# KamilSJaron/smudgeplot

Hardware: NVIDIA H100
Metric: k-mers/sec scanned (hetmers) at 1/2/4/8 H100; bit-exact .smu vs ref C (higher is better)
Workload: dtype u64

## Files before the change

### smudgeplot_b200/csrc/hm_symm.cu

```cuda
#include <cuda_runtime.h>
#include <stdint.h>
#include <stdio.h>
#include <stdlib.h>
#include <string.h>

#include "hetmers_b200.h"
#include "hm_internal.h"
#include "hm_device.cuh"

#define RS_THREADS 256
#define RS_EPT     8
#define RS_TILE    (RS_THREADS*RS_EPT)
#define RS_HALO    64
#define RS_WIN     (RS_TILE+2*RS_HALO)
#define RS_SCANCAP RS_HALO
#define RS_RUNCAP  (RS_HALO+1)
#define RS_LONGRUN 32
#ifndef RS_MINBLOCKS
#define RS_MINBLOCKS 5
#endif
#ifndef RS_STAGE
#define RS_STAGE   384
#endif

#define SY_STATUS_ASYMMETRIC 1ull
#define SY_STATUS_OVERFLOW   2ull

#define SY_HDR_CAND   0
#define SY_HDR_STATUS 1
#define SY_HDR_RUNS   2
#define SY_HDR_S      3
#define SY_HDR_PEND   4
#define SY_HDR_QUERY  5

struct SymmView
  { unsigned long long *cand_n;
    unsigned long long *status;
    uint32_t *bloom;
    uint32_t  seg_words;
    int       n_seg, self;
    uint64_t  first_key[HM_MAX_SHARDS];
    uint64_t *cand_key, *cand_lo, *cand_meta;
    unsigned long long cand_cap;
    unsigned long long *runs_n;
    uint64_t *runs;
    unsigned long long runs_cap;
    uint64_t *s_key, *s_lo;
    unsigned long long s_cap;
    const hm_stream_sview *sviews;
    uint64_t *pend, *pend_key, *pend_lo;
    uint64_t *q_key, *q_lo, *q_tag;
    unsigned long long pend_cap, q_cap;
  };

template <int KW>
__device__ __forceinline__ void bloom_slot(const SymmView &W, int seg, int kmer, uint64_t hi, uint64_t lo,
                                           uint64_t *&word, uint64_t &mask)
{ const int Pr = kmer >> 1, pup = kmer-Pr;
  uint64_t sfx;
  if (KW == 1)
    sfx = hi >> (64-2*kmer);
  else
    { const int sr = 128-2*kmer;
      sfx = sr == 0 ? lo : ((lo >> sr) | (hi << (64-sr)));
    }
  if (2*Pr < 64)
    sfx &= (((uint64_t) 1 << (2*Pr)) - 1);
  const uint64_t pfx = hi >> (64-2*pup);
  uint32_t h = ((uint32_t) sfx ^ (uint32_t) (sfx >> 32) * 0x85EBCA6Bu) * 0x9E3779B1u;
  uint32_t g = ((uint32_t) pfx ^ (uint32_t) (pfx >> 32) * 0xC2B2AE35u) * 0x27D4EB2Fu;
  h ^= h >> 15;
  word = (uint64_t *) (W.bloom + (size_t) seg * W.seg_words) + __umulhi(h * 0x2C1B3C6Du,W.seg_words >> 1);
  mask = (1ull << (g >> 26)) | (1ull << ((g >> 20) & 63)) | (1ull << ((g >> 14) & 63));
}

__device__ __forceinline__ uint64_t ld_keep(const uint64_t *p)
{ uint64_t v, pol;
  asm volatile("createpolicy.fractional.L2::evict_last.b64 %0, 1.0;" : "=l"(pol));
  asm volatile("ld.global.nc.L1::no_allocate.L2::cache_hint.u64 %0, [%1], %2;" : "=l"(v) : "l"(p), "l"(pol));
  return v;
}

__device__ __forceinline__ uint64_t ld_stream(const uint64_t *p)
{ uint64_t v, pol;
  asm volatile("createpolicy.fractional.L2::evict_first.b64 %0, 1.0;" : "=l"(pol));
  asm volatile("ld.global.nc.L1::no_allocate.L2::cache_hint.u64 %0, [%1], %2;" : "=l"(v) : "l"(p), "l"(pol));
  return v;
}

__device__ __forceinline__ void red_or64(uint64_t *p, uint64_t v)
{ asm volatile("red.global.relaxed.gpu.or.b64 [%0], %1;" :: "l"(__cvta_generic_to_global(p)), "l"(v) : "memory"); }

__device__ __forceinline__ int owner_of(const SymmView &W, uint64_t hi)
{ int r = 0;
  for (int s = 1; s < W.n_seg; s++)
    r += (hi >= W.first_key[s]);
  return r;
}

template <typename IdxT, int KW>
__device__ __noinline__ void neighbours_slow(const uint64_t *__restrict__ keys, const uint64_t *__restrict__ keys_lo,
                                             const uint16_t *__restrict__ cnt, const IdxT *__restrict__ bucket,
                                             int bshift, int kmer, int p0, int pup,
                                             uint64_t x, uint64_t xl, int cx,
                                             int &H, int &U, int64_t &part, int &ppos)
{ H = 0; U = 0; part = -1; ppos = 0;
  for (int p = p0; p < kmer; p++)
    { int b = base_at<KW>(x,xl,p);
      for (int c = 0; c < 4; c++)
        { if (c == b) continue;
          uint64_t y = x, yl = xl;
          set_base<KW>(y,yl,p,c);
          int64_t j = bucket_find<IdxT,KW>(keys,keys_lo,bucket,bshift,y,yl);
          if (j >= 0 && cx + (int) __ldg(cnt+j) <= HM_SMAX)
            { H += 1;
              if (p >= pup) U += 1;
              part = j; ppos = p;
            }
        }
    }
}


__device__ __forceinline__ uint64_t fp_mix(uint64_t hi, uint64_t lo, uint32_t c, uint64_t seed)
{ uint64_t v = (hi ^ seed) * 0xBF58476D1CE4E5B9ull;
  v ^= v >> 32;
  v = (v + lo + ((uint64_t) c << 40) + c) * 0x94D049BB133111EBull;
  v ^= v >> 29;
  v *= (seed | 1);
  v ^= v >> 32;
  return v;
}

template <int KW>
__global__ void __launch_bounds__(256)
symm_fingerprint_kernel(const uint64_t *__restrict__ keys, const uint64_t *__restrict__ keys_lo,
                        const uint16_t *__restrict__ cnt, int64_t i0, int64_t i1, int kmer,
                        uint64_t seed0, uint64_t seed1, unsigned long long *__restrict__ acc)
{ uint64_t a0 = 0, a1 = 0, a2 = 0, a3 = 0;
  const int64_t stride = (int64_t) gridDim.x * blockDim.x;
  for (int64_t i = i0 + (int64_t) blockIdx.x * blockDim.x + threadIdx.x; i < i1; i += stride)
    { uint64_t x = keys[i], xl = KW == 2 ? keys_lo[i] : 0, r, rl;
      uint32_t c = cnt[i];
      revcomp_kmer<KW>(x,xl,kmer,r,rl);
      a0 += fp_mix(x,xl,c,seed0);  a1 += fp_mix(x,xl,c,seed1);
      a2 += fp_mix(r,rl,c,seed0);  a3 += fp_mix(r,rl,c,seed1);
    }
  for (int o = 16; o > 0; o >>= 1)
    { a0 += __shfl_xor_sync(0xffffffffu,a0,o); a1 += __shfl_xor_sync(0xffffffffu,a1,o);
      a2 += __shfl_xor_sync(0xffffffffu,a2,o); a3 += __shfl_xor_sync(0xffffffffu,a3,o);
    }
  if ((threadIdx.x & 31) == 0)
    { atomicAdd(acc+0,(unsigned long long) a0); atomicAdd(acc+1,(unsigned long long) a1);
      atomicAdd(acc+2,(unsigned long long) a2); atomicAdd(acc+3,(unsigned long long) a3);
    }
}

extern "C" int hm_k_symm_fingerprint(const uint64_t *d_keys, const uint64_t *d_keys_lo, const uint16_t *d_cnt,
                                     int64_t i0, int64_t i1, int kmer, const uint64_t seed[2],
                                     uint64_t *d_acc, void *stream)
{ if (kmer < 1 || kmer > HM_MAX_KMER || (kmer > 32) != (d_keys_lo != NULL) || seed == NULL || d_acc == NULL)
    return hm_set_error(HM_EINVAL,"symm_fingerprint: bad arguments (k=%d)",kmer);
  if (i1 <= i0)
    return HM_OK;
  int64_t want = (i1-i0+255)/256;
  int     grid = (int) (want < 132*16 ? want : 132*16);
  if (kmer <= 32)
    symm_fingerprint_kernel<1><<<grid,256,0,(cudaStream_t) stream>>>
        (d_keys,NULL,d_cnt,i0,i1,kmer,seed[0],seed[1],(unsigned long long *) d_acc);
  else
    symm_fingerprint_kernel<2><<<grid,256,0,(cudaStream_t) stream>>>
        (d_keys,d_keys_lo,d_cnt,i0,i1,kmer,seed[0],seed[1],(unsigned long long *) d_acc);
// ... 43 lines not shown
  at = (at+255) & ~255ll;
  out->off_cand_key = at;   at += 8*cap;
  out->off_cand_lo = at;    at += (kmer > 32) ? 8*cap : 0;
  out->off_cand_meta = at;  at += 8*cap;
  out->cand_cap = cap;
  out->off_runs = at;       out->runs_cap = range/3 + 1024;   at += 8*out->runs_cap;
  out->n_seg = n_seg;
  out->range = range;
  out->bytes = (at+255) & ~255ll;
  return HM_OK;
}

static void bloom_window(cudaStream_t st, const void *base, size_t bytes, int on)
{ static int limit_set[64] = {0};
  static size_t max_win[64] = {0}, max_persist[64] = {0};
  int dev = 0;
  cudaGetDevice(&dev);
  if (dev < 0 || dev >= 64) return;
  if (!limit_set[dev])
    { cudaDeviceProp p;
      limit_set[dev] = 1;
      if (cudaGetDeviceProperties(&p,dev) == cudaSuccess)
        { max_win[dev] = (size_t) p.accessPolicyMaxWindowSize;
          max_persist[dev] = (size_t) p.persistingL2CacheMaxSize;
          if (max_persist[dev] > 0)
            cudaDeviceSetLimit(cudaLimitPersistingL2CacheSize,max_persist[dev]);
        }
      cudaGetLastError();
    }
  if (max_win[dev] == 0 || max_persist[dev] == 0)
    return;
  cudaStreamAttrValue a;
  memset(&a,0,sizeof(a));
  if (on)
    { size_t w = bytes < max_win[dev] ? bytes : max_win[dev];
      a.accessPolicyWindow.base_ptr  = (void *) base;
      a.accessPolicyWindow.num_bytes = w;
      a.accessPolicyWindow.hitRatio  = w <= max_persist[dev] ? 1.0f : (float) max_persist[dev] / (float) w;
      a.accessPolicyWindow.hitProp   = cudaAccessPropertyPersisting;
      a.accessPolicyWindow.missProp  = cudaAccessPropertyStreaming;
    }
  cudaStreamSetAttribute(st,cudaStreamAttributeAccessPolicyWindow,&a);
  cudaGetLastError();
}

static int l2_persist(void)
{ const char *e = getenv("HETMERS_L2_PERSIST");
  return (e == NULL || strcmp(e,"0") != 0);
}

static SymmView make_view(void *d_work, const hm_symm_layout *L, const hm_symm_shards *sh)
{ SymmView W;
  uint8_t *b = (uint8_t *) d_work;
  memset(&W,0,sizeof(W));
  W.cand_n    = (unsigned long long *) (b + L->off_header) + SY_HDR_CAND;
  W.status    = W.cand_n + SY_HDR_STATUS;
  W.bloom     = (uint32_t *) (b + L->off_bloom);
  W.seg_words = (uint32_t) L->seg_words;
  W.n_seg     = L->n_seg;
  W.self      = 0;
  if (sh != NULL && sh->n_seg > 1)
    { W.self = sh->self;
      for (int r = 0; r < sh->n_seg; r++) W.first_key[r] = sh->first_key[r];
    }
  W.cand_key  = (uint64_t *) (b + L->off_cand_key);
  W.cand_lo   = (uint64_t *) (b + L->off_cand_lo);
  W.cand_meta = (uint64_t *) (b + L->off_cand_meta);
  W.cand_cap  = (unsigned long long) L->cand_cap;
  W.runs_n    = W.cand_n + SY_HDR_RUNS;
  W.runs      = (uint64_t *) (b + L->off_runs);
  W.runs_cap  = (unsigned long long) L->runs_cap;
  return W;
}


template <int KW> struct RsSmem
  { uint64_t *key, *klo;
    uint16_t *cnt;
    uint64_t *ckey, *clo, *cmeta;
    uint16_t *t1;
    uint16_t *t2r;
  };

__device__ __forceinline__ uint64_t pack_meta(int cx, int cy, int pos, int yb)
{ return (uint64_t) cx | ((uint64_t) cy << 16) | ((uint64_t) pos << 32) | ((uint64_t) yb << 40); }

#ifdef RS_PROBE
__device__ int rs_probe_mode;
#define RS_PROBE_IS(m) (rs_probe_mode == (m))
#else
#define RS_PROBE_IS(m) false
#endif

template <int KW>
__device__ __forceinline__ void stage_candidates(const RsSmem<KW> &S, unsigned *s_nc, const SymmView &W,
                                                 bool emit, uint64_t x, uint64_t xl, uint64_t meta,
                                                 int lane, unsigned lt)
{ const unsigned bal = __ballot_sync(0xffffffffu,emit);
  if (bal == 0 || RS_PROBE_IS(4))
    return;
  unsigned base = 0;
  if (lane == 0)
    base = atomicAdd(s_nc,(unsigned) __popc(bal));
  base = __shfl_sync(0xffffffffu,base,0);
  const unsigned at = base + __popc(bal & lt);
  const bool     over = emit && (at >= RS_STAGE);
  if (emit && !over)
    { S.ckey[at] = x;
      if (KW == 2) S.clo[at] = xl;
      S.cmeta[at] = meta;
    }
  if (base + __popc(bal) <= RS_STAGE)
    return;
  const unsigned ob = __ballot_sync(0xffffffffu,over);
  unsigned long long g0 = 0;
  if (lane == 0)
    g0 = atomicAdd(W.cand_n,(unsigned long long) __popc(ob));
  g0 = __shfl_sync(0xffffffffu,g0,0) + (unsigned long long) __popc(ob & lt);
  if (over)
    { if (g0 < W.cand_cap)
        { W.cand_key[g0] = x;
          if (KW == 2) W.cand_lo[g0] = xl;
          W.cand_meta[g0] = meta;
        }
      else
        atomicOr(W.status,SY_STATUS_OVERFLOW);
    }
}

template <int KW>
__device__ __forceinline__ void s_push(const SymmView &W, uint64_t x, uint64_t xl)
{ const unsigned m = __activemask();
  const int      lane = threadIdx.x & 31, lead = __ffs(m)-1;
  unsigned long long at = 0;
  if (lane == lead)
    at = atomicAdd(W.cand_n + SY_HDR_S,(unsigned long long) __popc(m));
  at = __shfl_sync(m,at,lead) + (unsigned long long) __popc(m & ((1u << lane)-1));
  if (at < W.s_cap)
    { W.s_key[at] = x;
      if (KW == 2) W.s_lo[at] = xl;
    }
  else
    atomicOr(W.status,SY_STATUS_OVERFLOW);
}

template <int KW, bool SL>
__device__ __forceinline__ void bloom_insert(const SymmView &W, int kmer, uint64_t x, uint64_t xl)
{ uint64_t *word, mask;
  bloom_slot<KW>(W,W.self,kmer,x,xl,word,mask);
  if (!RS_PROBE_IS(3) || mask == (uint64_t) (uintptr_t) word)
    red_or64(word,mask);
  if (SL)
    s_push<KW>(W,x,xl);
}

template <typename IdxT, int KW, bool SL>
__global__ void __launch_bounds__(256)
runs_kernel(const uint64_t *__restrict__ keys, const uint64_t *__restrict__ keys_lo,
            const uint16_t *__restrict__ cnt, int64_t n, const IdxT *__restrict__ bucket, int bshift,
            int kmer, int64_t lo, int64_t hi, const SymmView W)
{ const int      Pr = kmer >> 1, pup = kmer-Pr, psh = 64-2*Pr;
  const uint64_t pmask = ~(uint64_t) 0 << psh;
  const unsigned FULL = 0xffffffffu;
  const int      lane = threadIdx.x & 31;
  const unsigned lt   = (1u << lane) - 1;
  unsigned long long nrl = *W.runs_n;
  if (nrl > W.runs_cap) nrl = W.runs_cap;
  const int64_t nr     = (int64_t) nrl;
  const int64_t stride = (int64_t) gridDim.x * blockDim.x;
  for (int64_t r0 = (int64_t) blockIdx.x * blockDim.x + threadIdx.x - lane; r0 < nr; r0 += stride)
    { const int64_t r = r0+lane;
      const bool    valid = (r < nr);
      int64_t  h = 0;
      uint64_t x0 = 0;
      if (valid)
        { h  = (int64_t) W.runs[r];
          x0 = __ldg(keys+h);
        }
      unsigned lb = __ballot_sync(FULL,valid);
      while (lb != 0)
        { const int     src = __ffs(lb)-1;
          lb &= lb-1;
          const int64_t hh = __shfl_sync(FULL,h,src);
          const uint64_t xx = __shfl_sync(FULL,x0,src);
          int64_t end = hh+1;
          while (true)
            { const int64_t t = end+lane;
              const bool same = (t < n) && (((__ldg(keys+t) ^ xx) & pmask) == 0);
              const unsigned sb = __ballot_sync(FULL,same);
              if (sb == FULL) { end += 32; continue; }
              end += __ffs(~sb)-1;
              break;
            }
          for (int64_t g0 = hh; g0 < end; g0 += 32)
            { const int64_t g = g0+lane;
              bool     emit = false;
              uint64_t x = 0, xl = 0, meta = 0;
              if (g < end && g >= lo && g < hi)
                { x = __ldg(keys+g);
                  if (KW == 2) xl = __ldg(keys_lo+g);
                  const int cx = __ldg(cnt+g);
                  int Hn, Un, ppos; int64_t part;
                  neighbours_slow<IdxT,KW>(keys,keys_lo,cnt,bucket,bshift,kmer,Pr,pup,x,xl,cx,Hn,Un,part,ppos);
                  if (Un > 0)
                    bloom_insert<KW,SL>(W,kmer,x,xl);
                  if (Hn == 1 && part > g)
                    { const uint64_t y = __ldg(keys+part), yl = KW == 2 ? __ldg(keys_lo+part) : 0;
                      const int cy = __ldg(cnt+part);
                      int Hy, Uy, py; int64_t party;
                      neighbours_slow<IdxT,KW>(keys,keys_lo,cnt,bucket,bshift,kmer,Pr,pup,y,yl,cy,Hy,Uy,party,py);
                      if (Hy == 1)
                        { emit = true;
                          meta = pack_meta(cx,cy,ppos,base_at<KW>(y,yl,ppos));
                        }
                    }
                }
              const unsigned eb = __ballot_sync(FULL,emit);
              if (eb != 0)
                { unsigned long long base = 0;
                  if (lane == 0)
                    base = atomicAdd(W.cand_n,(unsigned long long) __popc(eb));
                  base = __shfl_sync(FULL,base,0) + (unsigned long long) __popc(eb & lt);
                  if (emit)
                    { if (base < W.cand_cap)
                        { W.cand_key[base] = x;
                          if (KW == 2) W.cand_lo[base] = xl;
                          W.cand_meta[base] = meta;
                        }
                      else
                        atomicOr(W.status,SY_STATUS_OVERFLOW);
                    }
                }
            }
        }
    }
}

template <int KW> struct RunSfx    { typedef uint64_t T; };
template <>       struct RunSfx<1> { typedef uint32_t T; };

template <int KW>
__device__ __forceinline__ typename RunSfx<KW>::T run_sfx(uint64_t hi, uint64_t lo, int Pr)
{ if constexpr (KW == 1)
    return (uint32_t) ((hi << 2*Pr) >> 32);
  else
    return (hi << (2*Pr-32) << 32) | (lo >> (64-2*Pr));
}

template <typename T>
__device__ __forceinline__ bool one_base_in_run(T d, int Pr, int &pos)
{ const T u = (d | (d >> 1)) & (T) HM_M5;
  if constexpr (sizeof(T) == 4) pos = Pr + (__clz((int) d) >> 1);
  else                          pos = Pr + (__clzll((long long) d) >> 1);
  return (u & (u-1)) == 0;
}

template <int KW, bool SL, int LMAX>
__device__ __forceinline__ bool settle_members(const RsSmem<KW> &S, const SymmView &W, int kmer, int Pr, int pup,
                                               int h, int L, int a, bool in, bool own, int lane,
                                               uint64_t &x, uint64_t &xl, uint64_t &meta)
{ int Hx = 0, Ux = 0, part = 0, ppos = 0, cx = 0;
  if (in)
    { x  = S.key[h+a];
      xl = KW == 2 ? S.klo[h+a] : 0;
      cx = S.cnt[h+a];
      auto mate = [&](int b)
        { int pos;
          if (b < L && b != a && one_base_in_run(run_sfx<KW>(x ^ S.key[h+b],KW == 2 ? xl ^ S.klo[h+b] : 0,Pr),Pr,pos) &&
              cx + (int) S.cnt[h+b] <= HM_SMAX)
            { Hx += 1;
              if (pos >= pup) Ux += 1;
              part = b; ppos = pos;
            }
        };
      if constexpr (LMAX > 0)
        {
#pragma unroll
          for (int b = 0; b < LMAX; b++)
            mate(b);
        }
      else
        for (int b = 0; b < L; b++)
          mate(b);
      if (own && Ux > 0)
        bloom_insert<KW,SL>(W,kmer,x,xl);
    }
  const int pl = lane + part - a;
  int       Hy = __shfl_sync(0xffffffffu,Hx,pl & 31);
  if (!in || !own || Hx != 1 || part < a)
    return false;
  const uint64_t y = S.key[h+part], yl = KW == 2 ? S.klo[h+part] : 0;
  const int      cy = S.cnt[h+part];
  if (pl > 31)
    { Hy = 0;
      for (int b = 0; b < L; b++)
        { int pos;
          if (b != part && one_base_in_run(run_sfx<KW>(y ^ S.key[h+b],KW == 2 ? yl ^ S.klo[h+b] : 0,Pr),Pr,pos) &&
              cy + (int) S.cnt[h+b] <= HM_SMAX)
            Hy += 1;
        }
    }
  if (Hy != 1)
    return false;
  meta = pack_meta(cx,cy,ppos,base_at<KW>(y,yl,ppos));
  return true;
}

#ifdef RS_PROBE
#define RS_PHASES 6
#define RS_PROBE_SLOTS 1024
__device__ unsigned long long rs_probe_cycles[RS_PROBE_SLOTS*RS_PHASES];
#define RS_PROBE_TILE(b)  (rs_probe_mode == 2 ? (b) % 64 : (b))
#define RS_PROBE_START    long long rs_t = clock64(); unsigned long long rs_acc[RS_PHASES] = {0, 0, 0, 0, 0, 0};
#define RS_PROBE_MARK(ph) { const long long t_ = clock64(); rs_acc[ph] += (unsigned long long) (t_ - rs_t); rs_t = t_; }
#define RS_PROBE_FLUSH()  { if (lane == 0) _Pragma("unroll") for (int p_ = 0; p_ < RS_PHASES; p_++) \
                              atomicAdd(rs_probe_cycles + (blockIdx.x % RS_PROBE_SLOTS)*RS_PHASES + p_,rs_acc[p_]); }
#define RS_PROBE_LOADONLY() if (rs_probe_mode == 1) { RS_PROBE_FLUSH(); return; }

extern "C" int hm_probe_runscan(int mode, unsigned long long *cycles)
{ static unsigned long long rows[RS_PROBE_SLOTS*RS_PHASES];
  cudaError_t e = cudaDeviceSynchronize();
  if (e == cudaSuccess && cycles != NULL)
    { e = cudaMemcpyFromSymbol(rows,rs_probe_cycles,sizeof(rows));
      for (int p = 0; p < RS_PHASES; p++)
        { cycles[p] = 0;
          for (int r = 0; r < RS_PROBE_SLOTS; r++)
            cycles[p] += rows[r*RS_PHASES+p];
        }
    }
  memset(rows,0,sizeof(rows));
  if (e == cudaSuccess)
    e = cudaMemcpyToSymbol(rs_probe_cycles,rows,sizeof(rows));
  if (e == cudaSuccess)
    e = cudaMemcpyToSymbol(rs_probe_mode,&mode,sizeof(mode));
  return e == cudaSuccess ? HM_OK : hm_cuda_fail(e,"hm_probe_runscan");
}
#else
#define RS_PROBE_TILE(b)  (b)
#define RS_PROBE_START
#define RS_PROBE_MARK(ph)
#define RS_PROBE_FLUSH()
#define RS_PROBE_LOADONLY()
#endif

template <typename IdxT, int KW, bool SL>
__global__ void __launch_bounds__(RS_THREADS,RS_MINBLOCKS)
runscan_kernel(const uint64_t *__restrict__ keys, const uint64_t *__restrict__ keys_lo,
               const uint16_t *__restrict__ cnt, int64_t n, const IdxT *__restrict__ bucket, int bshift,
               int kmer, int64_t lo, int64_t hi, int64_t tile0, int use_tma, const SymmView W)
{ extern __shared__ __align__(128) uint8_t smem[];
  __shared__ __align__(8) uint64_t s_bar;
  __shared__ unsigned s_nc, s_nr, s_done;
  RsSmem<KW> S;
  S.key   = (uint64_t *) smem;
  S.klo   = S.key + (KW == 2 ? RS_WIN : 0);
  S.ckey  = S.key + KW*RS_WIN;
  S.clo   = S.ckey + (KW == 2 ? RS_STAGE : 0);
  S.cmeta = S.ckey + KW*RS_STAGE;
  S.cnt   = (uint16_t *) (S.cmeta + RS_STAGE);
  S.t1    = S.cnt + RS_WIN;
  S.t2r   = S.t1 + RS_TILE/2;

  const int      Pr   = kmer >> 1;
  const int      pup  = kmer - Pr;
  const int      psh  = 64-2*Pr;
  const uint64_t pmask = ~(uint64_t) 0 << psh;
  const unsigned FULL = 0xffffffffu;
  const int      lane = threadIdx.x & 31;
  const int      warp = threadIdx.x >> 5;
  const unsigned lt   = (1u << lane) - 1;
  RS_PROBE_START

  const int64_t T0 = (tile0 + RS_PROBE_TILE(blockIdx.x)) * RS_TILE;
  const int64_t ws = T0 - RS_HALO;
  const int64_t e0 = ws > 0 ? ws : 0;
  const int64_t e1 = T0+RS_TILE+RS_HALO < n ? T0+RS_TILE+RS_HALO : n;
  const int     v0 = (int) (e0-ws), v1 = (int) (e1-ws);

  const int m   = v1-v0;
  const int mt  = use_tma ? (m & ~7) : 0;
  if (threadIdx.x == 0)
    { s_nc = 0; s_nr = 0; s_done = 0;
      if (mt > 0)
        { mbar_init(&s_bar,1);
          fence_proxy_async_smem();
        }
    }
  __syncthreads();
  if (threadIdx.x == 0 && mt > 0)
    { mbar_arrive_expect_tx(&s_bar,(unsigned) (mt*(8*KW+2)));
      bulk_copy_g2s(S.key+v0,keys+e0,(unsigned) (8*mt),&s_bar);
      if (KW == 2)
        bulk_copy_g2s(S.klo+v0,keys_lo+e0,(unsigned) (8*mt),&s_bar);
      bulk_copy_g2s(S.cnt+v0,cnt+e0,(unsigned) (2*mt),&s_bar);
    }
  if (mt < m || v0 > 0 || v1 < RS_WIN)
    { for (int j = mt + threadIdx.x; j < m; j += RS_THREADS)
        { S.key[v0+j] = keys[e0+j];
          if (KW == 2) S.klo[v0+j] = keys_lo[e0+j];
          S.cnt[v0+j] = cnt[e0+j];
        }
      if (mt > 0)
        mbar_wait(&s_bar,0);
      __syncthreads();
      const uint64_t sa = ~S.key[v0], sb = ~S.key[v1-1];
      __syncthreads();
      for (int j = threadIdx.x; j < RS_WIN; j += RS_THREADS)
        if (j < v0)       S.key[j] = sa;
        else if (j >= v1) S.key[j] = sb;
      __syncthreads();
    }
  else
    mbar_wait(&s_bar,0);
  RS_PROBE_MARK(0)
  RS_PROBE_LOADONLY()

  const int wd0 = RS_HALO/32 + warp*RS_EPT;
  unsigned  eqw = 0;
#pragma unroll
  for (int t = 0; t < RS_EPT+2; t++)
    { const int i = (wd0-1+t)*32 + lane;
      bool eq;
      if (psh >= 32)
        { const uint32_t a = (uint32_t) (S.key[i] >> 32);
          uint32_t       b = __shfl_down_sync(FULL,a,1);
          if (lane == 31) b = (uint32_t) (S.key[i+1] >> 32);
          eq = (((a ^ b) >> (psh-32)) == 0);
        }
      else
        eq = (((S.key[i] ^ S.key[i+1]) & pmask) == 0);
      const unsigned bal = __ballot_sync(FULL,eq);
      if (lane == t) eqw = bal;
    }
  RS_PROBE_MARK(1)

  const int a0 = RS_HALO + (lo > T0 ? (int) (lo-T0 < RS_TILE ? lo-T0 : RS_TILE) : 0);
  const int a1 = RS_HALO + (hi-T0 < RS_TILE ? (int) (hi-T0) : RS_TILE);
  uint16_t *my1  = S.t1  + warp*(RS_TILE/2/(RS_THREADS/32));
  int n1, n3;
  { const unsigned P = __shfl_up_sync(FULL,eqw,1), N = __shfl_down_sync(FULL,eqw,1);
    unsigned m2 = 0, m3 = 0;
    const int wd = wd0-1+lane;
    if (lane >= 1 && lane <= RS_EPT)
      { const unsigned E = eqw;
        const unsigned em1 = (E << 1) | (P >> 31);
        const unsigned em2 = (E << 2) | (P >> 30);
        const unsigned ep1 = (E >> 1) | (N << 31);
        const int      s0  = wd*32;
        unsigned act = 0xffffffffu;
        if (s0 < a0)      act &= (a0-s0 >= 32) ? 0u : (0xffffffffu << (a0-s0));
        if (s0+32 > a1)   act &= (a1-s0 <= 0)  ? 0u : (0xffffffffu >> (s0+32-a1));
        const unsigned more = (em1 & E) | (E & ep1) | (em1 & em2);
        m2 = (E & ~em1 & ~ep1) & act;
        m3 = more & act & ~em1;
      }
    const int c2 = __popc(m2), c3 = __popc(m3);
    int pre2 = c2, pre3 = c3;
#pragma unroll
    for (int o = 1; o <= RS_EPT; o <<= 1)
      { int v2 = __shfl_up_sync(FULL,pre2,o), v3 = __shfl_up_sync(FULL,pre3,o);
        if (lane >= o) { pre2 += v2; pre3 += v3; }
      }
    n1 = __shfl_sync(FULL,pre2,RS_EPT);
    n3 = __shfl_sync(FULL,pre3,RS_EPT);
    int at = pre2-c2;
    while (m2 != 0)
      { my1[at++] = (uint16_t) (wd*32 + __ffs(m2)-1);
        m2 &= m2-1;
      }
    at = n1 + pre3-c3;
    while (m3 != 0)
      { my1[at++] = (uint16_t) (wd*32 + __ffs(m3)-1);
        m3 &= m3-1;
      }
  }
  __syncwarp();
  if (RS_PROBE_IS(5))
    n3 = 0;
  RS_PROBE_MARK(2)

  for (int i0 = 0; i0 < n1; i0 += 32)
    { const int i = i0+lane;
      bool     emit = false;
      uint64_t x = 0, xl = 0, meta = 0;
      if (i < n1)
        { const int w = my1[i];
          x = S.key[w];
          const uint64_t y = S.key[w+1];
          uint64_t yl = 0;
          if (KW == 2) { xl = S.klo[w]; yl = S.klo[w+1]; }
          const int cx = S.cnt[w], cy = S.cnt[w+1];
          int pos;
          if (one_base_in_run(run_sfx<KW>(x ^ y,xl ^ yl,Pr),Pr,pos) && cx+cy <= HM_SMAX)
            { emit = true;
              meta = pack_meta(cx,cy,pos,base_at<KW>(y,yl,pos));
              if (pos >= pup)
                { bloom_insert<KW,SL>(W,kmer,x,xl);
                  bloom_insert<KW,SL>(W,kmer,y,yl);
                }
            }
        }
      stage_candidates<KW>(S,&s_nc,W,emit,x,xl,meta,lane,lt);
    }
  RS_PROBE_MARK(3)

  const int b1 = hi-T0 < RS_TILE+RS_HALO ? RS_HALO + (int) (hi-T0) : RS_WIN;
  for (int i0 = 0; i0 < n3; i0 += 32)
    { const int i = i0+lane;
      const int h = i < n3 ? my1[n1+i] : 0;
      int       L = 0;
      {
        const int      t  = (h >> 5) - (wd0-1);
        const unsigned w0 = __shfl_sync(FULL,eqw,t & 31), w1 = __shfl_sync(FULL,eqw,(t+1) & 31);
        const unsigned up = __funnelshift_r(w0,w1,h & 31);
        if (i < n3)
          L = (~up != 0) ? __ffs((int) ~up) : 33;
      }
      const int Ls = L <= 8 ? L : 0;
      int inc = Ls;
#pragma unroll
      for (int o = 1; o < 32; o <<= 1)
        { const int v = __shfl_up_sync(FULL,inc,o);
          if (lane >= o) inc += v;
        }
      const int M = __shfl_sync(FULL,inc,31);
      for (int t0 = 0; t0 < M; t0 += 32)
        { const int t = t0+lane;
          int r = 0;
#pragma unroll
          for (int s = 16; s > 0; s >>= 1)
            if (__shfl_sync(FULL,inc,r+s-1) <= t) r += s;
          const int hr = __shfl_sync(FULL,h,r), Lr = __shfl_sync(FULL,Ls,r);
          const int a  = t - (__shfl_sync(FULL,inc,r) - Lr);
          bool     emit = false;
          uint64_t x = 0, xl = 0, meta = 0;
          emit = settle_members<KW,SL,8>(S,W,kmer,Pr,pup,hr,Lr,a,t < M,hr+a < b1,lane,x,xl,meta);
          stage_candidates<KW>(S,&s_nc,W,emit,x,xl,meta,lane,lt);
        }
      unsigned lb = __ballot_sync(FULL,L > 8);
      while (lb != 0)
        { const int src = __ffs(lb)-1;
          lb &= lb-1;
          const int hh = __shfl_sync(FULL,h,src);
          int       LL = __shfl_sync(FULL,L,src);
          if (LL > 32)
            { const uint64_t xh = S.key[hh];
              while (LL <= RS_RUNCAP)
                { const int      t = hh+LL+lane;
                  const unsigned sb = __ballot_sync(FULL,t < RS_WIN && ((S.key[t] ^ xh) & pmask) == 0);
                  if (sb != FULL) { LL += __ffs(~sb)-1; break; }
                  LL += 32;
                }
            }
          if (LL > RS_RUNCAP || hh+LL >= RS_WIN)
            { if (lane == 0)
                S.t2r[atomicAdd(&s_nr,1u)] = (uint16_t) hh;
              continue;
            }
          for (int a0 = 0; a0 < LL; a0 += 32)
            { const int a = a0+lane;
              bool     emit = false;
              uint64_t x = 0, xl = 0, meta = 0;
              emit = settle_members<KW,SL,0>(S,W,kmer,Pr,pup,hh,LL,a,a < LL,hh+a < b1,lane,x,xl,meta);
              stage_candidates<KW>(S,&s_nc,W,emit,x,xl,meta,lane,lt);
            }
        }
    }
  RS_PROBE_MARK(4)

  __syncwarp();
  unsigned last = 0;
  if (lane == 0)
    { __threadfence_block();
      last = (atomicAdd(&s_done,1u) == RS_THREADS/32-1);
    }
  last = __shfl_sync(FULL,last,0);
  if (!last || RS_PROBE_IS(4))
    { RS_PROBE_MARK(5) RS_PROBE_FLUSH() return; }
  __threadfence_block();
  const unsigned nr = s_nr;
  if (nr > 0)
    { unsigned long long rb = 0;
      if (lane == 0)
        rb = atomicAdd(W.runs_n,(unsigned long long) nr);
      rb = __shfl_sync(FULL,rb,0);
      for (unsigned i = lane; i < nr; i += 32)
        if (rb+i < W.runs_cap)
          W.runs[rb+i] = (uint64_t) (T0 + ((int) S.t2r[i] - RS_HALO));
        else
          atomicOr(W.status,SY_STATUS_OVERFLOW);
    }
  const unsigned nc = s_nc < RS_STAGE ? s_nc : RS_STAGE;
  if (nc == 0)
    { RS_PROBE_MARK(5) RS_PROBE_FLUSH() return; }
  unsigned long long base = 0;
  if (lane == 0)
    base = atomicAdd(W.cand_n,(unsigned long long) nc);
  base = __shfl_sync(FULL,base,0);
  for (unsigned i = lane; i < nc; i += 32)
    { unsigned long long at = base + i;
      if (at < W.cand_cap)
        { W.cand_key[at] = S.ckey[i];
          if (KW == 2) W.cand_lo[at] = S.clo[i];
          W.cand_meta[at] = S.cmeta[i];
        }
      else
        atomicOr(W.status,SY_STATUS_OVERFLOW);
    }
  RS_PROBE_MARK(5)
  RS_PROBE_FLUSH()
}

template <typename IdxT, int KW, bool SL>
__global__ void __launch_bounds__(RS_THREADS,RS_MINBLOCKS)
runscan_dense_kernel(const uint64_t *__restrict__ keys, const uint64_t *__restrict__ keys_lo,
                     const uint16_t *__restrict__ cnt, int64_t n, int kmer, int64_t lo, int64_t hi,
                     int64_t tile0, int use_tma, const SymmView W)
{ extern __shared__ __align__(128) uint8_t smem[];
  __shared__ __align__(8) uint64_t s_bar;
  __shared__ unsigned s_nc, s_nl, s_done;
  __shared__ unsigned s_eq[RS_WIN/32+1];
  RsSmem<KW> S;
  S.key   = (uint64_t *) smem;
  S.klo   = S.key + (KW == 2 ? RS_WIN : 0);
  S.ckey  = S.key + KW*RS_WIN;
  S.clo   = S.ckey + (KW == 2 ? RS_STAGE : 0);
  S.cmeta = S.ckey + KW*RS_STAGE;
  S.cnt   = (uint16_t *) (S.cmeta + RS_STAGE);
  S.t1    = S.cnt + RS_WIN;
  S.t2r   = S.t1 + RS_WIN;
  uint16_t *s_part = S.t2r + RS_TILE/8;
  unsigned *hu = (unsigned *) (s_part + RS_WIN);
  uint32_t *rem = hu + RS_WIN/2;

  const int      Pr   = kmer >> 1, pup = kmer - Pr, psh = 64-2*Pr;
  const uint64_t pmask = ~(uint64_t) 0 << psh;
  const unsigned FULL = 0xffffffffu;
  const int      lane = threadIdx.x & 31;
  const int      warp = threadIdx.x >> 5;
  const unsigned lt   = (1u << lane) - 1;

  const int64_t T0 = (tile0 + blockIdx.x) * RS_TILE;
  const int64_t ws = T0 - RS_HALO;
  const int64_t e0 = ws > 0 ? ws : 0;
  const int64_t e1 = T0+RS_TILE+RS_HALO < n ? T0+RS_TILE+RS_HALO : n;
  const int     v0 = (int) (e0-ws), v1 = (int) (e1-ws);

  const int m   = v1-v0;
  const int mt  = use_tma ? (m & ~7) : 0;
  if (threadIdx.x == 0)
    { s_nc = 0; s_nl = 0; s_done = 0;
      if (mt > 0)
        { mbar_init(&s_bar,1);
          fence_proxy_async_smem();
        }
    }
  for (int j = threadIdx.x; j < RS_WIN/2; j += RS_THREADS)
    hu[j] = 0;
  __syncthreads();
  if (threadIdx.x == 0 && mt > 0)
    { mbar_arrive_expect_tx(&s_bar,(unsigned) (mt*(8*KW+2)));
      bulk_copy_g2s(S.key+v0,keys+e0,(unsigned) (8*mt),&s_bar);
      if (KW == 2)
        bulk_copy_g2s(S.klo+v0,keys_lo+e0,(unsigned) (8*mt),&s_bar);
      bulk_copy_g2s(S.cnt+v0,cnt+e0,(unsigned) (2*mt),&s_bar);
    }
  if (mt < m || v0 > 0 || v1 < RS_WIN)
    { for (int j = mt + threadIdx.x; j < m; j += RS_THREADS)
        { S.key[v0+j] = keys[e0+j];
          if (KW == 2) S.klo[v0+j] = keys_lo[e0+j];
          S.cnt[v0+j] = cnt[e0+j];
        }
      if (mt > 0)
        mbar_wait(&s_bar,0);
      __syncthreads();
      const uint64_t sa = ~S.key[v0], sb = ~S.key[v1-1];
      __syncthreads();
      for (int j = threadIdx.x; j < RS_WIN; j += RS_THREADS)
        if (j < v0)       S.key[j] = sa;
        else if (j >= v1) S.key[j] = sb;
      __syncthreads();
    }
  else
    mbar_wait(&s_bar,0);

  const bool narrow = (KW == 1) && (kmer-Pr <= 16);
  for (int wd = warp; wd < RS_WIN/32; wd += RS_THREADS/32)
    { const int i = wd*32 + lane;
      bool eq = false;
      const uint64_t ki = S.key[i];
      if (i+1 < RS_WIN)
        eq = (((ki ^ S.key[i+1]) & pmask) == 0);
      if (narrow)
        rem[i] = (uint32_t) ((ki << (2*Pr)) >> 32);
      const unsigned bal = __ballot_sync(FULL,eq);
      if (lane == 0)
        s_eq[wd] = bal;
    }
  if (threadIdx.x == 0)
    s_eq[RS_WIN/32] = 0;
  __syncthreads();

  const int a0 = RS_HALO + (lo > T0 ? (int) (lo-T0 < RS_TILE ? lo-T0 : RS_TILE) : 0);
  const int a1 = RS_HALO + (hi-T0 < RS_TILE ? (int) (hi-T0) : RS_TILE);
  for (int i = threadIdx.x; i < RS_WIN; i += RS_THREADS)
    { const int      w = i >> 5, b = i & 31;
      const unsigned up = __funnelshift_r(s_eq[w],s_eq[w+1],b);
      const int      fwd = (~up == 0) ? 32 : __ffs((int) ~up)-1;
      int back = 0;
      if (i > 0)
        { const int      wq = (i-1) >> 5, bq = (i-1) & 31;
          const unsigned dn = __funnelshift_l(wq > 0 ? s_eq[wq-1] : 0u,s_eq[wq],31-bq);
          back = (~dn == 0) ? 32 : __clz((int) ~dn);
        }
      uint16_t mark = (uint16_t) fwd;
      if (back+fwd+1 > RS_LONGRUN)
        { mark = 0xffff;
          if (back == 0 && i >= a0 && i < a1)
            S.t2r[atomicAdd(&s_nl,1u)] = (uint16_t) i;
        }
      S.t1[i] = mark;
      s_part[i] = (uint16_t) i;
    }
  __syncthreads();

  for (int i = threadIdx.x; i < RS_WIN; i += RS_THREADS)
    { const int fwd = S.t1[i];
      if (fwd == 0 || fwd == 0xffff)
        continue;
      const int cx = S.cnt[i];
      if (narrow)
        { const uint32_t rx = rem[i];
          for (int j = i+1; j <= i+fwd; j++)
            { const uint32_t d = rx ^ rem[j];
              const uint32_t u = (d | (d>>1)) & 0x55555555u;
              if ((u & (u-1)) == 0 && cx + (int) S.cnt[j] <= HM_SMAX)
                { const int      pos = Pr + (__clz((int) d) >> 1);
                  const unsigned inc = 1u | (pos >= pup ? 0x100u : 0u);
                  atomicAdd(hu + (i>>1), inc << (16*(i&1)));
                  atomicAdd(hu + (j>>1), inc << (16*(j&1)));
                  s_part[i] = (uint16_t) j;
                  s_part[j] = (uint16_t) i;
                }
            }
        }
      else
        { const uint64_t x = S.key[i], xl = KW == 2 ? S.klo[i] : 0;
          for (int j = i+1; j <= i+fwd; j++)
            { int pos;
              if (one_base_apart<KW>(x,xl,S.key[j],KW == 2 ? S.klo[j] : 0,pos) && cx + (int) S.cnt[j] <= HM_SMAX)
                { const unsigned inc = 1u | (pos >= pup ? 0x100u : 0u);
                  atomicAdd(hu + (i>>1), inc << (16*(i&1)));
                  atomicAdd(hu + (j>>1), inc << (16*(j&1)));
                  s_part[i] = (uint16_t) j;
                  s_part[j] = (uint16_t) i;
                }
            }
        }
    }
  __syncthreads();

  for (int i0 = RS_HALO + (threadIdx.x & ~31); i0 < RS_HALO+RS_TILE; i0 += RS_THREADS)
    { const int i = i0+lane;
      bool     emit = false;
      uint64_t x = 0, xl = 0, meta = 0;
      if (i >= a0 && i < a1 && S.t1[i] != 0xffff)
        { const unsigned c = (hu[i>>1] >> (16*(i&1))) & 0xffffu;
          const int H = (int) (c & 0xff), U = (int) (c >> 8);
          if (H > 0)
            { x = S.key[i];
              if (KW == 2) xl = S.klo[i];
              if (U > 0)
                bloom_insert<KW,SL>(W,kmer,x,xl);
              const int j = s_part[i];
              if (H == 1 && j > i && ((hu[j>>1] >> (16*(j&1))) & 0xffu) == 1)
                { const uint64_t y = S.key[j], yl = KW == 2 ? S.klo[j] : 0;
                  int pos;
                  one_base_apart<KW>(x,xl,y,yl,pos);
                  emit = true;
                  meta = pack_meta(S.cnt[i],S.cnt[j],pos,base_at<KW>(y,yl,pos));
                }
            }
        }
      stage_candidates<KW>(S,&s_nc,W,emit,x,xl,meta,lane,lt);
    }

  __syncwarp();
  unsigned last = 0;
  if (lane == 0)
    { __threadfence_block();
      last = (atomicAdd(&s_done,1u) == RS_THREADS/32-1);
    }
  last = __shfl_sync(FULL,last,0);
  if (!last)
    return;
  __threadfence_block();
  const unsigned nr = s_nl;
  if (nr > 0)
    { unsigned long long rb = 0;
      if (lane == 0)
        rb = atomicAdd(W.runs_n,(unsigned long long) nr);
      rb = __shfl_sync(FULL,rb,0);
      for (unsigned i = lane; i < nr; i += 32)
        if (rb+i < W.runs_cap)
          W.runs[rb+i] = (uint64_t) (T0 + ((int) S.t2r[i] - RS_HALO));
        else
          atomicOr(W.status,SY_STATUS_OVERFLOW);
    }
  const unsigned nc = s_nc < RS_STAGE ? s_nc : RS_STAGE;
  if (nc == 0)
    return;
  unsigned long long base = 0;
  if (lane == 0)
    base = atomicAdd(W.cand_n,(unsigned long long) nc);
  base = __shfl_sync(FULL,base,0);
  for (unsigned i = lane; i < nc; i += 32)
    { unsigned long long at = base + i;
      if (at < W.cand_cap)
        { W.cand_key[at] = S.ckey[i];
          if (KW == 2) W.cand_lo[at] = S.clo[i];
          W.cand_meta[at] = S.cmeta[i];
        }
      else
        atomicOr(W.status,SY_STATUS_OVERFLOW);
    }
}

template <typename I, int K> struct Inst { typedef I IdxT; static constexpr int KW = K; };

template <class F>
static cudaError_t dispatch(int kmer, int idx64, F f)
{ if (kmer <= 32)
    return idx64 ? f(Inst<uint64_t,1>()) : f(Inst<uint32_t,1>());
  return idx64 ? f(Inst<uint64_t,2>()) : f(Inst<uint32_t,2>());
}

template <typename IdxT, int KW, bool SL = false>
static cudaError_t launch_runscan(const uint64_t *keys, const uint64_t *keys_lo, const uint16_t *cnt, int64_t n,
                                  const void *bucket, int bits, int kmer, int64_t lo, int64_t hi,
                                  const SymmView &W, cudaStream_t st)
{ static int configured[64] = {0};
  int dev = 0;
  cudaGetDevice(&dev);
  int64_t tile0 = lo/RS_TILE, tile1 = (hi+RS_TILE-1)/RS_TILE;
  int     tma   = ((((uintptr_t) keys) | ((uintptr_t) cnt) | ((uintptr_t) (keys_lo ? keys_lo : keys))) & 15) == 0;
  const int   Pr  = kmer >> 1;
  double      lam = (2*Pr >= 62) ? 0.0 : (double) n / (double) ((uint64_t) 1 << (2*Pr));
  bool        dense = (lam > 0.6);
  const char *force = getenv("HETMERS_RUNSCAN");
  if (force != NULL && strcmp(force,"dense") == 0)  dense = true;
  if (force != NULL && strcmp(force,"sparse") == 0) dense = false;
  cudaError_t e;
  if (dense)
    { size_t smem = (size_t) RS_WIN*(8*KW+2) + (size_t) RS_STAGE*8*(KW+1) +
                    2*(size_t) (RS_WIN+RS_TILE/8+RS_WIN) + 4*(size_t) (RS_WIN/2+RS_WIN);
      if (smem > 48*1024 && (dev >= 64 || !(configured[dev] & 2)))
        { e = cudaFuncSetAttribute(runscan_dense_kernel<IdxT,KW,SL>,cudaFuncAttributeMaxDynamicSharedMemorySize,(int) smem);
          if (e != cudaSuccess) return e;
          if (dev < 64) configured[dev] |= 2;
        }
      runscan_dense_kernel<IdxT,KW,SL><<<(unsigned) (tile1-tile0),RS_THREADS,smem,st>>>
          (keys,keys_lo,cnt,n,kmer,lo,hi,tile0,tma,W);
    }
  else
    { size_t smem = (size_t) RS_WIN*(8*KW+2) + (size_t) RS_STAGE*8*(KW+1) +
                    2*(size_t) (RS_TILE/2+RS_TILE/2);
      if (smem > 48*1024 && (dev >= 64 || !(configured[dev] & 1)))
        { e = cudaFuncSetAttribute(runscan_kernel<IdxT,KW,SL>,cudaFuncAttributeMaxDynamicSharedMemorySize,(int) smem);
          if (e != cudaSuccess) return e;
          if (dev < 64) configured[dev] |= 1;
        }
      runscan_kernel<IdxT,KW,SL><<<(unsigned) (tile1-tile0),RS_THREADS,smem,st>>>
          (keys,keys_lo,cnt,n,(const IdxT *) bucket,64-bits,kmer,lo,hi,tile0,tma,W);
    }
  return cudaGetLastError();
}

template <typename IdxT, int KW, bool SL = false>
static cudaError_t launch_runs(const uint64_t *keys, const uint64_t *keys_lo, const uint16_t *cnt, int64_t n,
                               const void *bucket, int bits, int kmer, int64_t lo, int64_t hi,
                               const SymmView &W, cudaStream_t st)
{
  int dev = 0, sms = 132;
  cudaGetDevice(&dev);
  cudaDeviceGetAttribute(&sms,cudaDevAttrMultiProcessorCount,dev);
  int64_t want = ((hi-lo)/64+255)/256;
  int     grid = (int) (want < sms*8 ? (want > 0 ? want : 1) : sms*8);
  runs_kernel<IdxT,KW,SL><<<grid,256,0,st>>>(keys,keys_lo,cnt,n,(const IdxT *) bucket,64-bits,kmer,lo,hi,W);
  return cudaGetLastError();
}

extern "C" int hm_k_symm_runscan(const uint64_t *d_keys, const uint64_t *d_keys_lo, const uint16_t *d_cnt, int64_t n,
                                 const void *d_bucket, int bits, int idx64, int kmer, int64_t lo, int64_t hi,
                                 void *d_work, const hm_symm_layout *layout, const hm_symm_shards *shards,
                                 void *stream)
{ if (kmer < HM_SYMM_MIN_KMER || kmer > HM_MAX_KMER)
    return hm_set_error(HM_EUNSUPPORTED,"symmetric scan needs %d <= k <= %d (k=%d)",HM_SYMM_MIN_KMER,HM_MAX_KMER,kmer);
  if (lo < 0 || hi > n || lo > hi || bits < 1 || bits > 30 || d_work == NULL || layout == NULL)
    return hm_set_error(HM_EINVAL,"symm_runscan: bad range [%lld,%lld) of %lld or bits %d",
                        (long long) lo,(long long) hi,(long long) n,bits);
  if ((kmer > 32) != (d_keys_lo != NULL))
    return hm_set_error(HM_EINVAL,"symm_runscan: second key word array %s for k=%d",
                        d_keys_lo ? "given" : "missing",kmer);
  if ((shards != NULL && shards->n_seg > 1) != (layout->n_seg > 1) ||
      (shards != NULL && shards->n_seg > 1 && (shards->n_seg != layout->n_seg || shards->self < 0 ||
                                               shards->self >= shards->n_seg)))
    return hm_set_error(HM_EINVAL,"symm_runscan: shard table does not match the work-area layout");
  cudaStream_t st = (cudaStream_t) stream;
  SymmView W = make_view(d_work,layout,shards);
  HM_CUDA(cudaMemsetAsync(W.cand_n,0,256,st));
  HM_CUDA(cudaMemsetAsync(W.bloom + (size_t) W.self*W.seg_words,0,sizeof(uint32_t)*(size_t) W.seg_words,st));
  if (l2_persist())
    bloom_window(st,W.bloom,sizeof(uint32_t)*(size_t) W.seg_words*(size_t) W.n_seg,1);
  if (hi == lo)
    return HM_OK;
  cudaError_t e = dispatch(kmer,idx64,[&](auto I)
    { return launch_runscan<typename decltype(I)::IdxT,decltype(I)::KW>(d_keys,d_keys_lo,d_cnt,n,d_bucket,bits,kmer,
                                                                       lo,hi,W,st); });
  if (e != cudaSuccess)
    return hm_cuda_fail(e,"runscan_kernel");
  return HM_OK;
}

extern "C" int hm_k_symm_runs(const uint64_t *d_keys, const uint64_t *d_keys_lo, const uint16_t *d_cnt, int64_t n,
                              const void *d_bucket, int bits, int idx64, int kmer, int64_t lo, int64_t hi,
                              void *d_work, const hm_symm_layout *layout, const hm_symm_shards *shards,
                              void *stream)
{ if (kmer < HM_SYMM_MIN_KMER || kmer > HM_MAX_KMER || d_work == NULL || layout == NULL ||
      (kmer > 32) != (d_keys_lo != NULL) || lo < 0 || hi > n || lo > hi)
    return hm_set_error(HM_EINVAL,"symm_runs: bad arguments");
  if (hi == lo)
    return HM_OK;
  cudaStream_t st = (cudaStream_t) stream;
  SymmView W = make_view(d_work,layout,shards);
  cudaError_t e = dispatch(kmer,idx64,[&](auto I)
    { return launch_runs<typename decltype(I)::IdxT,decltype(I)::KW>(d_keys,d_keys_lo,d_cnt,n,d_bucket,bits,kmer,
                                                                    lo,hi,W,st); });
  if (e != cudaSuccess)
    return hm_cuda_fail(e,"runs_kernel");
  return HM_OK;
}


#define RV_TS   192
#define RV_TM   96
#define RV_TROW 97
#define RV_THREADS 1024
#ifndef RV_ILP
#define RV_ILP 2
#endif
#define RV_QCAP  (32*(RV_ILP+1))
#define RV_PROBE 4
#define RV_HA    (1ull << 48)
#define RV_HB    (1ull << 49)

#ifdef RESOLVE_PROBE
#define RVP_BINS 50
#define RVP_CAND 0
#define RVP_HA   1
#define RVP_HB   2
#define RVP_HAB  3
#define RVP_GEN  4
#define RVP_HIST 5
#define RVP_NCTR (RVP_HIST+RVP_BINS)
__device__ unsigned long long rvp_ctr[RVP_NCTR];
__device__ int rvp_mode;
#define RVP_MODE rvp_mode
#define RVP_COUNT(i,v) { if (rvp_mode == 3) atomicAdd(rvp_ctr+(i),(unsigned long long) (v)); }
#define RVP_BUCKET(sz) RVP_COUNT(RVP_HIST + ((sz) < RVP_BINS-1 ? (int) (sz) : RVP_BINS-1),1)

extern "C" int hm_probe_resolve(int mode, unsigned long long *ctr)
{ static unsigned long long rows[RVP_NCTR];
  cudaError_t e = cudaDeviceSynchronize();
  if (e == cudaSuccess && ctr != NULL)
    { e = cudaMemcpyFromSymbol(rows,rvp_ctr,sizeof(rows));
      memcpy(ctr,rows,sizeof(rows));
    }
  memset(rows,0,sizeof(rows));
// ... 999 lines not shown
```

Baseline: 129.1 billion.

## Replace last-warp tail flush with block-wide cooperative candidate and run flush

The per-tile output flush used to be done by whichever warp finished last, detected with a shared atomic counter, and that single warp wrote all staged candidates and runs to global memory. Now all threads meet at a __syncthreads, thread 0 reserves global slots for candidates and runs in one step, every thread preloads its share of staged candidates into registers, and the whole block writes them out. This spreads the serial single-warp tail across 256 threads, at the cost of a full block barrier. RS_MINBLOCKS is also raised from 5 to 6, which tightens the register cap in exchange for higher occupancy. The probe instrumentation gains extra phase and lifetime columns.

```diff
diff --git a/smudgeplot_b200/csrc/hm_symm.cu b/smudgeplot_b200/csrc/hm_symm.cu
--- a/smudgeplot_b200/csrc/hm_symm.cu
+++ b/smudgeplot_b200/csrc/hm_symm.cu
@@ -17,7 +17,7 @@
 #define RS_RUNCAP  (RS_HALO+1)
 #define RS_LONGRUN 32
 #ifndef RS_MINBLOCKS
-#define RS_MINBLOCKS 5
+#define RS_MINBLOCKS 6
 #endif
 #ifndef RS_STAGE
 #define RS_STAGE   384
@@ -367,6 +367,53 @@
     red_or64(word,mask);
   if (SL)
     s_push<KW>(W,x,xl);
+}
+
+#define RS_FLUSH ((RS_STAGE+RS_THREADS-1)/RS_THREADS)
+struct RsFlush { uint64_t key[RS_FLUSH], lo[RS_FLUSH], meta[RS_FLUSH]; };
+
+template <int KW>
+__device__ __forceinline__ void flush_reserve(const RsSmem<KW> &S, unsigned long long *s_cb,
+                                              unsigned long long *s_rb, const SymmView &W,
+                                              unsigned nc, unsigned nr, RsFlush &F)
+{ if (threadIdx.x == 0)
+    { if (nc > 0) *s_cb = atomicAdd(W.cand_n,(unsigned long long) nc);
+      if (nr > 0) *s_rb = atomicAdd(W.runs_n,(unsigned long long) nr);
+    }
+#pragma unroll
+  for (int j = 0; j < RS_FLUSH; j++)
+    { const unsigned i = threadIdx.x + j*RS_THREADS;
+      if (i < nc)
+        { F.key[j] = S.ckey[i];
+          if (KW == 2) F.lo[j] = S.clo[i];
+          F.meta[j] = S.cmeta[i];
+        }
+    }
+}
+
+template <int KW>
+__device__ __forceinline__ void flush_store(const RsSmem<KW> &S, unsigned long long cb, unsigned long long rb,
+                                            const SymmView &W, unsigned nc, unsigned nr, int64_t T0,
+                                            const RsFlush &F)
+{
+#pragma unroll
+  for (int j = 0; j < RS_FLUSH; j++)
+    { const unsigned i = threadIdx.x + j*RS_THREADS;
+      if (i < nc)
+        { if (cb+i < W.cand_cap)
+            { W.cand_key[cb+i] = F.key[j];
+              if (KW == 2) W.cand_lo[cb+i] = F.lo[j];
+              W.cand_meta[cb+i] = F.meta[j];
+            }
+          else
+            atomicOr(W.status,SY_STATUS_OVERFLOW);
+        }
+    }
+  for (unsigned i = threadIdx.x; i < nr; i += RS_THREADS)
+    if (rb+i < W.runs_cap)
+      W.runs[rb+i] = (uint64_t) (T0 + ((int) S.t2r[i] - RS_HALO));
+    else
+      atomicOr(W.status,SY_STATUS_OVERFLOW);
 }
 
 template <typename IdxT, int KW, bool SL>
@@ -522,25 +569,36 @@
 }
 
 #ifdef RS_PROBE
-#define RS_PHASES 6
+#define RS_PHASES 8
+#define RS_COLS   (RS_PHASES+3)
 #define RS_PROBE_SLOTS 1024
-__device__ unsigned long long rs_probe_cycles[RS_PROBE_SLOTS*RS_PHASES];
+__device__ unsigned long long rs_probe_cycles[RS_PROBE_SLOTS*RS_COLS];
 #define RS_PROBE_TILE(b)  (rs_probe_mode == 2 ? (b) % 64 : (b))
-#define RS_PROBE_START    long long rs_t = clock64(); unsigned long long rs_acc[RS_PHASES] = {0, 0, 0, 0, 0, 0};
+#define RS_PROBE_START    __shared__ long long rs_t0, rs_t1; \
+                          long long rs_t = clock64(); unsigned long long rs_acc[RS_PHASES] = {0, 0, 0, 0, 0, 0, 0, 0}; \
+                          if (threadIdx.x == 0) rs_t0 = rs_t;
 #define RS_PROBE_MARK(ph) { const long long t_ = clock64(); rs_acc[ph] += (unsigned long long) (t_ - rs_t); rs_t = t_; }
+#define RS_PROBE_LANDED() if (threadIdx.x == 0) rs_t1 = clock64();
+#define RS_PROBE_ALLDONE  const long long rs_t2 = clock64();
+#define RS_PROBE_ROW      (rs_probe_cycles + (blockIdx.x % RS_PROBE_SLOTS)*RS_COLS)
 #define RS_PROBE_FLUSH()  { if (lane == 0) _Pragma("unroll") for (int p_ = 0; p_ < RS_PHASES; p_++) \
-                              atomicAdd(rs_probe_cycles + (blockIdx.x % RS_PROBE_SLOTS)*RS_PHASES + p_,rs_acc[p_]); }
+                              atomicAdd(RS_PROBE_ROW + p_,rs_acc[p_]); }
+#define RS_PROBE_LIFE()   { const long long t3_ = clock64(); \
+                            if (threadIdx.x == 0) { atomicAdd(RS_PROBE_ROW + RS_PHASES,  (unsigned long long) (rs_t1 - rs_t0)); \
+                                             atomicAdd(RS_PROBE_ROW + RS_PHASES+1,(unsigned long long) (rs_t2 - rs_t1)); \
+                                             atomicAdd(RS_PROBE_ROW + RS_PHASES+2,(unsigned long long) (t3_ - rs_t2)); } }
 #define RS_PROBE_LOADONLY() if (rs_probe_mode == 1) { RS_PROBE_FLUSH(); return; }
+#define RS_PROBE_NOTAIL()   if (rs_probe_mode == 6) { RS_PROBE_FLUSH(); return; }
 
 extern "C" int hm_probe_runscan(int mode, unsigned long long *cycles)
-{ static unsigned long long rows[RS_PROBE_SLOTS*RS_PHASES];
+{ static unsigned long long rows[RS_PROBE_SLOTS*RS_COLS];
   cudaError_t e = cudaDeviceSynchronize();
   if (e == cudaSuccess && cycles != NULL)
     { e = cudaMemcpyFromSymbol(rows,rs_probe_cycles,sizeof(rows));
-      for (int p = 0; p < RS_PHASES; p++)
+      for (int p = 0; p < RS_COLS; p++)
         { cycles[p] = 0;
           for (int r = 0; r < RS_PROBE_SLOTS; r++)
-            cycles[p] += rows[r*RS_PHASES+p];
+            cycles[p] += rows[r*RS_COLS+p];
         }
     }
   memset(rows,0,sizeof(rows));
@@ -554,8 +612,12 @@
 #define RS_PROBE_TILE(b)  (b)
 #define RS_PROBE_START
 #define RS_PROBE_MARK(ph)
+#define RS_PROBE_LANDED()
+#define RS_PROBE_ALLDONE
 #define RS_PROBE_FLUSH()
+#define RS_PROBE_LIFE()
 #define RS_PROBE_LOADONLY()
+#define RS_PROBE_NOTAIL()
 #endif
 
 template <typename IdxT, int KW, bool SL>
@@ -565,7 +627,8 @@
                int kmer, int64_t lo, int64_t hi, int64_t tile0, int use_tma, const SymmView W)
 { extern __shared__ __align__(128) uint8_t smem[];
   __shared__ __align__(8) uint64_t s_bar;
-  __shared__ unsigned s_nc, s_nr, s_done;
+  __shared__ unsigned s_nc, s_nr;
+  __shared__ unsigned long long s_base[2];
   RsSmem<KW> S;
   S.key   = (uint64_t *) smem;
   S.klo   = S.key + (KW == 2 ? RS_WIN : 0);
@@ -595,7 +658,7 @@
   const int m   = v1-v0;
   const int mt  = use_tma ? (m & ~7) : 0;
   if (threadIdx.x == 0)
-    { s_nc = 0; s_nr = 0; s_done = 0;
+    { s_nc = 0; s_nr = 0;
       if (mt > 0)
         { mbar_init(&s_bar,1);
           fence_proxy_async_smem();
@@ -628,6 +691,7 @@
   else
     mbar_wait(&s_bar,0);
   RS_PROBE_MARK(0)
+  RS_PROBE_LANDED()
   RS_PROBE_LOADONLY()
 
   const int wd0 = RS_HALO/32 + warp*RS_EPT;
@@ -782,47 +846,23 @@
         }
     }
   RS_PROBE_MARK(4)
-
-  __syncwarp();
-  unsigned last = 0;
-  if (lane == 0)
-    { __threadfence_block();
-      last = (atomicAdd(&s_done,1u) == RS_THREADS/32-1);
-    }
-  last = __shfl_sync(FULL,last,0);
-  if (!last || RS_PROBE_IS(4))
-    { RS_PROBE_MARK(5) RS_PROBE_FLUSH() return; }
-  __threadfence_block();
-  const unsigned nr = s_nr;
-  if (nr > 0)
-    { unsigned long long rb = 0;
-      if (lane == 0)
-        rb = atomicAdd(W.runs_n,(unsigned long long) nr);
-      rb = __shfl_sync(FULL,rb,0);
-      for (unsigned i = lane; i < nr; i += 32)
-        if (rb+i < W.runs_cap)
-          W.runs[rb+i] = (uint64_t) (T0 + ((int) S.t2r[i] - RS_HALO));
-        else
-          atomicOr(W.status,SY_STATUS_OVERFLOW);
-    }
-  const unsigned nc = s_nc < RS_STAGE ? s_nc : RS_STAGE;
-  if (nc == 0)
-    { RS_PROBE_MARK(5) RS_PROBE_FLUSH() return; }
-  unsigned long long base = 0;
-  if (lane == 0)
-    base = atomicAdd(W.cand_n,(unsigned long long) nc);
-  base = __shfl_sync(FULL,base,0);
-  for (unsigned i = lane; i < nc; i += 32)
-    { unsigned long long at = base + i;
-      if (at < W.cand_cap)
-        { W.cand_key[at] = S.ckey[i];
-          if (KW == 2) W.cand_lo[at] = S.clo[i];
-          W.cand_meta[at] = S.cmeta[i];
-        }
-      else
-        atomicOr(W.status,SY_STATUS_OVERFLOW);
-    }
+  RS_PROBE_NOTAIL()
+
+  __syncthreads();
   RS_PROBE_MARK(5)
+  RS_PROBE_ALLDONE
+  if (RS_PROBE_IS(4))
+    { RS_PROBE_FLUSH() return; }
+  const unsigned nc = s_nc < RS_STAGE ? s_nc : RS_STAGE, nr = s_nr;
+  if (nc == 0 && nr == 0)
+    { RS_PROBE_MARK(6) RS_PROBE_LIFE() RS_PROBE_FLUSH() return; }
+  RsFlush F;
+  flush_reserve<KW>(S,&s_base[0],&s_base[1],W,nc,nr,F);
+  __syncthreads();
+  RS_PROBE_MARK(6)
+  flush_store<KW>(S,s_base[0],s_base[1],W,nc,nr,T0,F);
+  RS_PROBE_MARK(7)
+  RS_PROBE_LIFE()
   RS_PROBE_FLUSH()
 }
 
@@ -833,7 +873,8 @@
                      int64_t tile0, int use_tma, const SymmView W)
 { extern __shared__ __align__(128) uint8_t smem[];
   __shared__ __align__(8) uint64_t s_bar;
-  __shared__ unsigned s_nc, s_nl, s_done;
+  __shared__ unsigned s_nc, s_nl;
+  __shared__ unsigned long long s_base[2];
   __shared__ unsigned s_eq[RS_WIN/32+1];
   RsSmem<KW> S;
   S.key   = (uint64_t *) smem;
@@ -864,7 +905,7 @@
   const int m   = v1-v0;
   const int mt  = use_tma ? (m & ~7) : 0;
   if (threadIdx.x == 0)
-    { s_nc = 0; s_nl = 0; s_done = 0;
+    { s_nc = 0; s_nl = 0;
       if (mt > 0)
         { mbar_init(&s_bar,1);
           fence_proxy_async_smem();
@@ -1000,45 +1041,14 @@
       stage_candidates<KW>(S,&s_nc,W,emit,x,xl,meta,lane,lt);
     }
 
-  __syncwarp();
-  unsigned last = 0;
-  if (lane == 0)
-    { __threadfence_block();
-      last = (atomicAdd(&s_done,1u) == RS_THREADS/32-1);
-    }
-  last = __shfl_sync(FULL,last,0);
-  if (!last)
+  __syncthreads();
+  const unsigned nc = s_nc < RS_STAGE ? s_nc : RS_STAGE, nr = s_nl;
+  if (nc == 0 && nr == 0)
     return;
-  __threadfence_block();
-  const unsigned nr = s_nl;
-  if (nr > 0)
-    { unsigned long long rb = 0;
-      if (lane == 0)
-        rb = atomicAdd(W.runs_n,(unsigned long long) nr);
-      rb = __shfl_sync(FULL,rb,0);
-      for (unsigned i = lane; i < nr; i += 32)
-        if (rb+i < W.runs_cap)
-          W.runs[rb+i] = (uint64_t) (T0 + ((int) S.t2r[i] - RS_HALO));
-        else
-          atomicOr(W.status,SY_STATUS_OVERFLOW);
-    }
-  const unsigned nc = s_nc < RS_STAGE ? s_nc : RS_STAGE;
-  if (nc == 0)
-    return;
-  unsigned long long base = 0;
-  if (lane == 0)
-    base = atomicAdd(W.cand_n,(unsigned long long) nc);
-  base = __shfl_sync(FULL,base,0);
-  for (unsigned i = lane; i < nc; i += 32)
-    { unsigned long long at = base + i;
-      if (at < W.cand_cap)
-        { W.cand_key[at] = S.ckey[i];
-          if (KW == 2) W.cand_lo[at] = S.clo[i];
-          W.cand_meta[at] = S.cmeta[i];
-        }
-      else
-        atomicOr(W.status,SY_STATUS_OVERFLOW);
-    }
+  RsFlush F;
+  flush_reserve<KW>(S,&s_base[0],&s_base[1],W,nc,nr,F);
+  __syncthreads();
+  flush_store<KW>(S,s_base[0],s_base[1],W,nc,nr,T0,F);
 }
 
 template <typename I, int K> struct Inst { typedef I IdxT; static constexpr int KW = K; };
```

New measurement: 137.4 billion (median of 6 runs). 6.4% higher.
